# Samirez/Visual_odometry

Hardware: AMD Instinct MI355X
Metric: frame-pairs/sec (1280x720, 2000 ORB feats) (higher is better)
Workload: dtype u8+f32+f64; 1 GPU; seeded synthetic 1280x720 drone flight (256 distinct rendered views, closed loop), 2000 ORB features/frame, 8 levels = BASELINE config 2; chunk of 257 consecutive frames -> 256 pairs (k, k+1) per GPU per step, each frame detected once; detector=orb, distinct_rendered_frames=256, pair_stride=1, contexts_per_gpu=3, keypoint_order=cv2, poly_solver=fast, matcher=crosscheck, matcher_kernel=mfma_fp4, ransac=5-point, conf 0.99, 1 px, seed 2^64-1, <=1000 iters, parallelism=single GPU, pairs_ok_last_step=256

## Files before the change

include/vo_hip.h:

```cpp
#ifndef VO_HIP_H
#define VO_HIP_H
#include <stddef.h>
#include <stdint.h>

#ifdef __cplusplus
extern "C" {
#endif

#define VO_MAX_LEVELS 16

#define VO_OK                 0
#define VO_WARN_CAPACITY      1
#define VO_ERR_INVALID       -1
#define VO_ERR_HIP           -2
#define VO_ERR_TOO_FEW       -3
#define VO_ERR_NO_MODEL      -4
#define VO_ERR_NOT_CONFIGURED -5
#define VO_ERR_UNSUPPORTED    -7
#define VO_ERR_AMBIGUOUS      -6

typedef struct vo_ctx vo_ctx;

typedef struct {
    int32_t nfeatures;
// ... 26 lines not shown

int vo_set_pnp_refine(vo_ctx* ctx, int kind);

int vo_match_hamming(vo_ctx* ctx, const uint8_t* q, int nq, const uint8_t* t, int nt, int cross_check,
                     int32_t* qidx, int32_t* tidx, float* dist, int32_t* n_out);

int vo_match_l2(vo_ctx* ctx, const float* q, int nq, const float* t, int nt, int dim, int cross_check,
                int32_t* qidx, int32_t* tidx, float* dist, int32_t* n_out);

int vo_knn2_ratio_hamming(vo_ctx* ctx, const uint8_t* q, int nq, const uint8_t* t, int nt, double ratio,
                          int32_t* qidx, int32_t* tidx, float* dist, int32_t* n_out);
int vo_knn2_hamming(vo_ctx* ctx, const uint8_t* q, int nq, const uint8_t* t, int nt, int32_t* idx, float* dist);
int vo_knn2_l2(vo_ctx* ctx, const float* q, int nq, const float* t, int nt, int dim, int32_t* idx, float* dist);
int vo_knn2_ratio_l2(vo_ctx* ctx, const float* q, int nq, const float* t, int nt, int dim, double ratio,
                     int32_t* qidx, int32_t* tidx, float* dist, int32_t* n_out);

int vo_find_essential_ransac(vo_ctx* ctx, const double* p1, const double* p2, int M, const double* K,
                             double prob, double thresh_px, int max_iters, uint64_t seed,
                             double* E, uint8_t* mask, int32_t* n_inl, int32_t* n_models);

int vo_recover_pose(vo_ctx* ctx, const double* E, const double* p1, const double* p2, int M, const double* K,
                    double dist_thresh, double* R, double* t, uint8_t* mask, int32_t* n_good);

int vo_triangulate(vo_ctx* ctx, const double* P1, const double* P2, const double* x1, const double* x2,
                   int M, double* X);

int64_t vo_packed_pyramid_bytes(int h, int w, const vo_orb_params* params);
int vo_stage_pyramid(vo_ctx* ctx, const uint8_t* img, int h, int w, int channels, int row_stride,
                     const vo_orb_params* params, uint8_t* out_packed);
int vo_stage_fast_scores(vo_ctx* ctx, const uint8_t* img, int h, int w, int channels, int row_stride,
                         const vo_orb_params* params, uint8_t* out_packed);
int vo_stage_blur(vo_ctx* ctx, const uint8_t* img, int h, int w, int channels, int row_stride,
                  const vo_orb_params* params, uint8_t* out_packed);
int vo_stage_retain_best(vo_ctx* ctx, const float* response, int n, int n_points, int32_t* order, int32_t* n_out);
int vo_stage_five_point(vo_ctx* ctx, const double* x1, const double* x2, double* E , int32_t* n_models);

typedef struct {
    int32_t match_mode;
    double  ratio;
    double  ransac_prob;
    double  ransac_thresh;
    int32_t ransac_max_iters;
    uint64_t ransac_seed;
    double  pose_dist_thresh;
    int32_t want_points;
} vo_pair_opts;

typedef struct {
    int32_t n_kp1, n_kp2, n_match, n_inl, n_good, status, ransac_iters, reserved;
    double  R[9], t[3], E[9];
} vo_pair_result;

int vo_batch_configure(vo_ctx* ctx, int h, int w, const vo_orb_params* params, int max_frames, int max_pairs);
int vo_frames_upload(vo_ctx* ctx, const uint8_t* frames, int F, int row_stride, int64_t frame_stride, int first_slot);
int vo_frames_upload_async(vo_ctx* ctx, const uint8_t* frames, int F, int row_stride, int64_t frame_stride, int first_slot);
int vo_frames_upload_color(vo_ctx* ctx, const uint8_t* frames, int F, int channels, int row_stride,
                           int64_t frame_stride, int first_slot);
int vo_frames_detect(vo_ctx* ctx, int first_slot, int F);
int vo_frames_detect_async(vo_ctx* ctx, int first_slot, int F);
int vo_batch_kp_capacity(vo_ctx* ctx);
int  vo_host_alloc(size_t bytes, void** out);
void vo_host_free(void* p);
int vo_frame_features(vo_ctx* ctx, int slot, float* kp_xy, float* kp_size, float* kp_angle, float* kp_response,
                      int32_t* kp_octave, uint8_t* desc, int cap, int32_t* n_out);
int vo_pairs_run(vo_ctx* ctx, const int32_t* pair_slots, int B, const double* K, const vo_pair_opts* opts,
                 vo_pair_result* results, double* X, int32_t x_cap);
// ... 118 lines not shown
```

visual_odometry_amd/_lib.py:

```python
from __future__ import annotations

import ctypes as C
import os

import numpy as np

_HERE = os.path.dirname(os.path.abspath(__file__))
LIB_PATH = os.environ.get("VO_HIP_LIBRARY") or os.path.join(_HERE, "libvo_hip.so")

VO_OK, VO_WARN_CAPACITY = 0, 1
VO_ERR_INVALID, VO_ERR_HIP, VO_ERR_TOO_FEW, VO_ERR_NO_MODEL, VO_ERR_NOT_CONFIGURED, VO_ERR_AMBIGUOUS = -1, -2, -3, -4, -5, -6
VO_ERR_UNSUPPORTED = -7
VO_STAGE_COUNT = 28
VO_COMM_ID_BYTES, VO_RECORD_DOUBLES = 128, 16
VO_BA_MAX_CAMERAS, VO_BA_MAX_FREE = 64, 16


class OrbParams(C.Structure):
    _fields_ = [("nfeatures", C.c_int32), ("scale_factor", C.c_float), ("nlevels", C.c_int32),
                ("edge_threshold", C.c_int32), ("first_level", C.c_int32), ("wta_k", C.c_int32),
                ("score_type", C.c_int32), ("patch_size", C.c_int32), ("fast_threshold", C.c_int32)]


class SiftParams(C.Structure):
# ... 9 lines not shown

class BaOpts(C.Structure):
    _fields_ = [("iterations", C.c_int32), ("reserved", C.c_int32), ("huber_delta", C.c_double)]


class SlamOpts(C.Structure):
    _fields_ = [("pnp_iterations", C.c_int32), ("reproj_err", C.c_double), ("confidence", C.c_double), ("seed", C.c_uint64),
                ("max_point_norm", C.c_double), ("ba_iterations", C.c_int32), ("huber_delta", C.c_double),
                ("free_cameras", C.c_int32), ("filter_threshold", C.c_double), ("max_cameras", C.c_int32),
                ("snapshot_pair", C.c_int32), ("snapshot_stage", C.c_int32)]


PAIR_RESULT_DTYPE = np.dtype([("n_kp1", "<i4"), ("n_kp2", "<i4"), ("n_match", "<i4"), ("n_inl", "<i4"),
                              ("n_good", "<i4"), ("status", "<i4"), ("ransac_iters", "<i4"), ("reserved", "<i4"),
                              ("R", "<f8", (9,)), ("t", "<f8", (3,)), ("E", "<f8", (9,))], align=True)

_P = C.c_void_p
_SIGS = {
    "vo_create": (C.c_int, [C.c_int, C.POINTER(_P)]),
    "vo_destroy": (None, [_P]),
    "vo_last_error": (C.c_char_p, [_P]),
    "vo_version": (C.c_int, []),
    "vo_orb_detect_and_compute": (C.c_int, [_P, _P, C.c_int, C.c_int, C.c_int, C.c_int, _P, _P, _P, _P, _P, _P, _P, C.c_int, _P]),
    "vo_match_hamming": (C.c_int, [_P, _P, C.c_int, _P, C.c_int, C.c_int, _P, _P, _P, _P]),
    "vo_match_l2": (C.c_int, [_P, _P, C.c_int, _P, C.c_int, C.c_int, C.c_int, _P, _P, _P, _P]),
    "vo_knn2_ratio_hamming": (C.c_int, [_P, _P, C.c_int, _P, C.c_int, C.c_double, _P, _P, _P, _P]),
    "vo_find_essential_ransac": (C.c_int, [_P, _P, _P, C.c_int, _P, C.c_double, C.c_double, C.c_int, C.c_uint64, _P, _P, _P, _P]),
    "vo_recover_pose": (C.c_int, [_P, _P, _P, _P, C.c_int, _P, C.c_double, _P, _P, _P, _P]),
    "vo_triangulate": (C.c_int, [_P, _P, _P, _P, _P, C.c_int, _P]),
    "vo_packed_pyramid_bytes": (C.c_int64, [C.c_int, C.c_int, _P]),
    "vo_stage_pyramid": (C.c_int, [_P, _P, C.c_int, C.c_int, C.c_int, C.c_int, _P, _P]),
    "vo_stage_fast_scores": (C.c_int, [_P, _P, C.c_int, C.c_int, C.c_int, C.c_int, _P, _P]),
    "vo_stage_blur": (C.c_int, [_P, _P, C.c_int, C.c_int, C.c_int, C.c_int, _P, _P]),
    "vo_stage_five_point": (C.c_int, [_P, _P, _P, _P, _P]),
    "vo_batch_configure": (C.c_int, [_P, C.c_int, C.c_int, _P, C.c_int, C.c_int]),
    "vo_frames_upload": (C.c_int, [_P, _P, C.c_int, C.c_int, C.c_int64, C.c_int]),
    "vo_frames_upload_async": (C.c_int, [_P, _P, C.c_int, C.c_int, C.c_int64, C.c_int]),
    "vo_frames_upload_color": (C.c_int, [_P, _P, C.c_int, C.c_int, C.c_int, C.c_int64, C.c_int]),
    "vo_frames_detect": (C.c_int, [_P, C.c_int, C.c_int]),
    "vo_frames_detect_async": (C.c_int, [_P, C.c_int, C.c_int]),
    "vo_batch_kp_capacity": (C.c_int, [_P]),
    "vo_host_alloc": (C.c_int, [C.c_size_t, C.POINTER(_P)]),
    "vo_host_free": (None, [_P]),
    "vo_frame_features": (C.c_int, [_P, C.c_int, _P, _P, _P, _P, _P, _P, C.c_int, _P]),
    "vo_pairs_run": (C.c_int, [_P, _P, C.c_int, _P, _P, _P, _P, C.c_int32]),
    "vo_pairs_run_async": (C.c_int, [_P, _P, C.c_int, _P, _P, _P, _P, C.c_int32]),
    "vo_sync": (C.c_int, [_P]),
    "vo_set_matcher_kernel": (C.c_int, [_P, C.c_int]),
    "vo_set_poly_solver": (C.c_int, [_P, C.c_int]),
    "vo_set_pnp_refine": (C.c_int, [_P, C.c_int]),
    "vo_set_keypoint_order": (C.c_int, [_P, C.c_int]),
    "vo_stage_retain_best": (C.c_int, [_P, _P, C.c_int, C.c_int, _P, _P]),
    "vo_detect_after": (C.c_int, [_P, _P]),
    "vo_knn2_hamming": (C.c_int, [_P, _P, C.c_int, _P, C.c_int, _P, _P]),
    "vo_knn2_l2": (C.c_int, [_P, _P, C.c_int, _P, C.c_int, C.c_int, _P, _P]),
    "vo_knn2_ratio_l2": (C.c_int, [_P, _P, C.c_int, _P, C.c_int, C.c_int, C.c_double, _P, _P, _P, _P]),
    "vo_tracks_pnp_batch": (C.c_int, [_P, C.c_int, _P, C.c_int, C.c_double, C.c_double, C.c_uint64, C.c_double, _P, _P, _P, _P, _P]),
    "vo_slam_chain": (C.c_int, [_P, C.c_int, _P, _P, _P, _P, _P, _P, _P, _P, _P, _P, _P, _P, _P]),
    "vo_slam_map_size": (C.c_int, [_P, C.c_int, _P, _P, _P]),
    "vo_slam_map": (C.c_int, [_P, C.c_int, _P, _P, _P, _P, _P, _P, _P, _P]),
    "vo_slam_chains": (C.c_int, [_P, C.c_int, _P, _P, _P, C.c_int, _P, _P, _P, _P, _P, _P, _P, _P, _P, _P, _P]),
    "vo_slam_chains_map_size": (C.c_int, [_P, C.c_int, C.c_int, _P, _P, _P]),
    "vo_slam_chains_map": (C.c_int, [_P, C.c_int, C.c_int, _P, _P, _P, _P, _P, _P, _P, _P]),
    "vo_comm_unique_id": (C.c_int, [_P]),
    "vo_comm_init": (C.c_int, [_P, _P, C.c_int, C.c_int]),
    "vo_comm_destroy": (C.c_int, [_P]),
# ... 205 lines not shown
```

visual_odometry_amd/csrc/orb_kernels.hip:

```cpp
#include "vo_internal.h"
#include <type_traits>
#include <float.h>
#include <stdlib.h>

__constant__ int8_t c_pattern[256 * 4] = {
#include "orb_pattern.inc"
};
__constant__ int c_umax[16] = {15, 15, 15, 15, 14, 14, 14, 13, 13, 12, 11, 10, 9, 8, 6, 3};
__constant__ int c_gauss7[7] = {18, 34, 49, 55, 49, 34, 18};


typedef short vo_s16x2 __attribute__((ext_vector_type(2)));
typedef unsigned short vo_u16x2 __attribute__((ext_vector_type(2)));
__device__ __forceinline__ uint32_t pk_sub16(uint32_t a, uint32_t b)
{
    return __builtin_bit_cast(uint32_t, __builtin_bit_cast(vo_s16x2, a) - __builtin_bit_cast(vo_s16x2, b));
}
__device__ __forceinline__ uint32_t pk_add16(uint32_t a, uint32_t b)
{
    return __builtin_bit_cast(uint32_t, __builtin_bit_cast(vo_s16x2, a) + __builtin_bit_cast(vo_s16x2, b));
}
__device__ __forceinline__ uint32_t pk_min16(uint32_t a, uint32_t b)
{
    return __builtin_bit_cast(uint32_t, __builtin_elementwise_min(__builtin_bit_cast(vo_s16x2, a), __builtin_bit_cast(vo_s16x2, b)));
// ... 114 lines not shown
        const int dx = dx0 + b;
        uint32_t v = 0;
        if (dx < dst.w) {
            uint32_t h0, h1;
            if (dx < tab.min_x)       { h0 = (uint32_t)s0[0] << 8; h1 = (uint32_t)s1[0] << 8; }
            else if (dx >= tab.max_x) { h0 = (uint32_t)s0[src.w - 1] << 8; h1 = (uint32_t)s1[src.w - 1] << 8; }
            else {
                const int xo = tab.xofs[dx];
                const uint32_t c1 = tab.xc1[dx], c0 = 256 - c1;
                h0 = c0 * s0[xo] + c1 * s0[xo + 1];
                h1 = c0 * s1[xo] + c1 * s1[xo + 1];
            }
            v = edge ? (h0 + 128u) >> 8 : (h0 * w0 + h1 * w1 + 32768u) >> 16;
            v = v > 255u ? 255u : v;
        }
        out |= v << (8 * b);
    }
    *(uint32_t*)(dp + (size_t)dy * dst.stride + dx0) = out;
}

template <int I, int N, typename F>
__device__ __forceinline__ void unroll_while(int n, F& f)
{
    if constexpr (I < N) {
        if (I < n) { f(std::integral_constant<int, I>{}); unroll_while<I + 1, N>(n, f); }
    }
}

#ifndef RS3_AHEAD
#define RS3_AHEAD 4
#endif
__global__ __launch_bounds__(RS2_THREADS) void k_resize_direct(uint8_t* pyr, int frame_bytes, LevelGeom src, LevelGeom dst, ResizeTab tab)
{
    const int f = blockIdx.z, tid = threadIdx.x, lane = tid & 63, wave = __builtin_amdgcn_readfirstlane(tid >> 6);
    const int tiles_x = (dst.w + RS2_WW - 1) / RS2_WW;
    const int bid = xcd_tile(blockIdx.x, gridDim.x);
    const int tx = bid % tiles_x, ty = bid / tiles_x;
    const int x0 = tx * RS2_WW, y0 = ty * RS2_TH;
    const int dy0 = y0 + wave * RS2_WH, dy1 = min(dy0 + RS2_WH, dst.h);
    if (dy0 >= dst.h) return;
    const uint8_t* sp = pyr + (size_t)f * frame_bytes + src.off;
    const int dx = x0 + 4 * lane;
    int o[4], c1[4];
#pragma unroll
    for (int i = 0; i < 4; i++) { const int xi = min(dx + i, dst.w - 1); o[i] = tab.xofs[xi]; c1[i] = tab.xc1[xi]; }
    static_assert(RS2_WH <= 64, "one lane per destination row of the strip");
    const int li = min(dy0 + lane, dst.h - 1);
    const int yo_l = tab.yofs[li];
    const uint32_t yw1 = tab.yc1[li];
    const int yc_l = (int)((256u - yw1) | (yw1 << 16));
    const int yo_first = __builtin_amdgcn_readlane(yo_l, 0), yo_last = __builtin_amdgcn_readlane(yo_l, dy1 - 1 - dy0);
    const int base = o[0] & ~3, sh = o[0] - base;
    const uint32_t q1 = (uint32_t)(o[1] - o[0]), q2 = (uint32_t)(o[2] - o[0]), q3 = (uint32_t)(o[3] - o[0]);
    const uint32_t sel_ae = 0x0c000c00u | (q2 << 16), sel_ao = 0x0c000c00u | q1 | (q3 << 16);
    const uint32_t sel_be = sel_ae + 0x00010001u, sel_bo = sel_ao + 0x00010001u;
    const uint32_t c1e = (uint32_t)c1[0] | ((uint32_t)c1[2] << 16), c1o = (uint32_t)c1[1] | ((uint32_t)c1[3] << 16);
    const int r_first = yo_first, r_end = yo_last + 2;
    static_assert((RS2_WH * 127 + 99) / 100 + 3 <= 32, "the emit mask of a strip fits 32 bits");
    uint32_t emask = dy0 + lane < dy1 ? 1u << (yo_l + 1 - r_first) : 0u;
#pragma unroll
    for (int d = 1; d < RS2_WH; d <<= 1) emask |= (uint32_t)__shfl_xor((int)emask, d, 64);
    emask = (uint32_t)__builtin_amdgcn_readfirstlane((int)emask);
    const __amdgpu_buffer_rsrc_t drs = __builtin_amdgcn_make_buffer_rsrc(pyr + (size_t)f * frame_bytes + dst.off, 0, dst.stride * dst.h, 0x00020000);
    uint32_t out = (uint32_t)(dy0 * dst.stride + dx);
    const bool col_ok = dx < dst.stride;
    const int hmax = src.h - 1;
    uint32_t w[RS3_AHEAD][3];
#pragma unroll
    for (int u = 0; u < RS3_AHEAD; u++) {
        const uint32_t* q = (const uint32_t*)(sp + ((uint32_t)(min(r_first + u, hmax) * src.stride) + (uint32_t)base));
        w[u][0] = q[0]; w[u][1] = q[1]; w[u][2] = q[2];
    }
    int dyi = 0;
    uint32_t pe = 0, po = 0;
    const int nrows = r_end - r_first;
    constexpr int RS3_MAXR = (RS2_WH * 127 + 99) / 100 + 3;
    auto row = [&](auto ic) {
        constexpr int i = decltype(ic)::value, u = i % RS3_AHEAD;
        const uint32_t w0 = w[u][0], w1 = w[u][1], w2 = w[u][2];
        {
            const uint32_t* q = (const uint32_t*)(sp + ((uint32_t)(min(r_first + i + RS3_AHEAD, hmax) * src.stride) + (uint32_t)base));
            w[u][0] = q[0]; w[u][1] = q[1]; w[u][2] = q[2];
        }
        const uint32_t x0w = __builtin_amdgcn_alignbyte(w1, w0, (uint32_t)sh), x1w = __builtin_amdgcn_alignbyte(w2, w1, (uint32_t)sh);
        const uint32_t a_e = __builtin_amdgcn_perm(x1w, x0w, sel_ae), a_o = __builtin_amdgcn_perm(x1w, x0w, sel_ao);
        const uint32_t b_e = __builtin_amdgcn_perm(x1w, x0w, sel_be), b_o = __builtin_amdgcn_perm(x1w, x0w, sel_bo);
        const vo_u16x2 h_e = __builtin_bit_cast(vo_u16x2, c1e) * __builtin_bit_cast(vo_u16x2, pk_sub16(b_e, a_e)) + __builtin_bit_cast(vo_u16x2, a_e << 8);
        const vo_u16x2 h_o = __builtin_bit_cast(vo_u16x2, c1o) * __builtin_bit_cast(vo_u16x2, pk_sub16(b_o, a_o)) + __builtin_bit_cast(vo_u16x2, a_o << 8);
        const uint32_t ce = __builtin_bit_cast(uint32_t, h_e), co = __builtin_bit_cast(uint32_t, h_o);
        {
            const bool emit = emask & 1u;
            emask >>= 1;
            const vo_u16x2 wv = __builtin_bit_cast(vo_u16x2, __builtin_amdgcn_readlane(yc_l, dyi));
            const uint32_t d0 = __builtin_amdgcn_udot2(__builtin_bit_cast(vo_u16x2, __builtin_amdgcn_perm(ce, pe, 0x05040100u)), wv, 32768u, false);
            const uint32_t d2 = __builtin_amdgcn_udot2(__builtin_bit_cast(vo_u16x2, __builtin_amdgcn_perm(ce, pe, 0x07060302u)), wv, 32768u, false);
            const uint32_t d1 = __builtin_amdgcn_udot2(__builtin_bit_cast(vo_u16x2, __builtin_amdgcn_perm(co, po, 0x05040100u)), wv, 32768u, false);
            const uint32_t d3 = __builtin_amdgcn_udot2(__builtin_bit_cast(vo_u16x2, __builtin_amdgcn_perm(co, po, 0x07060302u)), wv, 32768u, false);
            const uint32_t t01 = __builtin_amdgcn_perm(d1, d0, 0x0c0c0602u), t23 = __builtin_amdgcn_perm(d3, d2, 0x0c0c0602u);
            __builtin_amdgcn_raw_buffer_store_b32(__builtin_amdgcn_perm(t23, t01, 0x05040100u), drs, col_ok && emit ? out : 0xfffffff0u, 0, 0);
            out += emit ? (uint32_t)dst.stride : 0u;
            dyi += emit ? 1 : 0;
        }
        pe = ce; po = co;
    };
    unroll_while<0, RS3_MAXR>(nrows, row);
}

void launch_resize(hipStream_t s, uint8_t* pyr, const PyrGeom& g, int level, const ResizeTab& tab, int F)
{
    const LevelGeom& d = g.lv[level];
    if (tab.direct) {
        dim3 grid(((d.w + RS2_WW - 1) / RS2_WW) * ((d.h + RS2_TH - 1) / RS2_TH), 1, F);
        hipLaunchKernelGGL(k_resize_direct, grid, dim3(RS2_THREADS), 0, s, pyr, g.frame_bytes, g.lv[level - 1], d, tab);
        return;
// ... 1084 lines not shown
        if (EDGE) { bd_fix(a0, a1, a2, e); bd_fix(b0, b1, b2, e); }
        bd_hpass(a0, a1, a2, h0); bd_hpass(b0, b1, b2, h1);
#pragma unroll
        for (int c = 0; c < 4; c++) q[c] = h0[c] | (h1[c] << 16);
    };
#pragma unroll
    for (int u = 0; u < BD_AHEAD; u++) fetch(u, W[u]);
#pragma unroll
    for (int k = 0; k < 3; k++) {
        hstep(W[k % BD_AHEAD], Q[k % 4]);
        fetch(k + BD_AHEAD, W[k % BD_AHEAD]);
    }
    uint32_t orow = (uint32_t)(y0 * lv.stride);
    for (int m0 = 0; m0 < nsteps; m0 += 4) {
#pragma unroll
        for (int j = 0; j < 4; j++) {
            const int m = m0 + j;
            if (m >= nsteps) break;
            constexpr int K0 = 3;
            const int ki = (K0 + j) % 4, wi = (K0 + j) % BD_AHEAD;
            hstep(W[wi], Q[ki]);
            fetch(K0 + m + BD_AHEAD, W[wi]);
            const uint32_t r0 = bd_vrow<false>(Q[(ki + 1) % 4], Q[(ki + 2) % 4], Q[(ki + 3) % 4], Q[ki]);
            const uint32_t r1 = bd_vrow<true>(Q[(ki + 1) % 4], Q[(ki + 2) % 4], Q[(ki + 3) % 4], Q[ki]);
            __builtin_amdgcn_raw_buffer_store_b32(r0, drs, col_ok ? (uint32_t)x + orow : 0xfffffff0u, 0, 0);
            __builtin_amdgcn_raw_buffer_store_b32(r1, drs, col_ok && 2 * m + 1 < nout ? (uint32_t)x + orow + (uint32_t)lv.stride : 0xfffffff0u, 0, 0);
            orow += 2u * (uint32_t)lv.stride;
        }
    }
}

__global__ __launch_bounds__(256) void k_blur_direct(const uint8_t* pyr, uint8_t* blur, PyrGeom g, int total)
{
    const int f = blockIdx.y, lane = threadIdx.x & 63, wave = __builtin_amdgcn_readfirstlane(threadIdx.x >> 6);
    const int wt = xcd_tile(blockIdx.x, gridDim.x) * 4 + wave;
    if (wt >= total) return;
    int l = 0, first = 0;
    for (;;) {
        const int nt = ((g.lv[l].stride + 255) / 256) * ((g.lv[l].h + BD_R - 1) / BD_R);
        if (wt < first + nt || l + 1 == g.nlevels) break;
        first += nt; l++;
    }
    const LevelGeom lv = g.lv[l];
    const int ntx = (lv.stride + 255) / 256, tile = wt - first;
    const int x0 = (tile % ntx) * 256, y0 = (tile / ntx) * BD_R;
    const int x = x0 + 4 * lane;
    const uint8_t* img = pyr + (size_t)f * g.frame_bytes + lv.off;
    const int xb = min(max(x - 4, 0), lv.stride - 12);
    BdEdge e;
    e.left = x0 == 0; e.right = x0 + 256 + 8 > lv.w;
    e.shl = x == 0; e.shr = x - 4 > lv.stride - 12 && x < lv.stride;
    {
        const int d = lv.w - x;
        e.s1 = d == 1 ? 0x01020304u : d == 2 ? 0x03040504u : d == 3 ? 0x05060504u : 0x07060504u;
        e.s2 = d == 2 ? 0x0c0c0c02u : d == 3 ? 0x0c0c0304u : 0x0c040506u;
        e.s3 = d == 5 ? 0x01020304u : d == 6 ? 0x03040504u : 0x07060504u;
        e.use_t = d >= 2 && d <= 4;
    }
    const __amdgpu_buffer_rsrc_t drs = __builtin_amdgcn_make_buffer_rsrc(blur + (size_t)f * g.frame_bytes + lv.off, 0, lv.stride * lv.h, 0x00020000);
    const bool col_ok = x < lv.stride;
    const int nout = min(BD_R, lv.h - y0);
    const int nsteps = (nout + 1) / 2;
    const bool inside = y0 >= 3 && y0 - 3 + 2 * (nsteps + 3 + BD_AHEAD) <= lv.h, edge = e.left || e.right;
    if (inside && !edge) bd_strip<true, false>(img, lv, drs, x, xb, y0, nout, nsteps, col_ok, e);
    else if (inside) bd_strip<true, true>(img, lv, drs, x, xb, y0, nout, nsteps, col_ok, e);
    else if (!edge) bd_strip<false, false>(img, lv, drs, x, xb, y0, nout, nsteps, col_ok, e);
    else bd_strip<false, true>(img, lv, drs, x, xb, y0, nout, nsteps, col_ok, e);
}

void launch_blur(hipStream_t s, const uint8_t* pyr, uint8_t* blur, const PyrGeom& g, int F)
{
    bool direct = true;
    int total = 0;
    for (int l = 0; l < g.nlevels; l++) {
        direct = direct && g.lv[l].w >= 16 && g.lv[l].h >= 8;
        total += ((g.lv[l].stride + 255) / 256) * ((g.lv[l].h + BD_R - 1) / BD_R);
    }
    if (direct) { hipLaunchKernelGGL(k_blur_direct, dim3((total + 3) / 4, F), dim3(256), 0, s, pyr, blur, g, total); return; }
    hipLaunchKernelGGL(k_blur, dim3(g.btiles_total, F), dim3(256), 0, s, pyr, blur, g);
}

__device__ __forceinline__ uint32_t brief_expand4(uint32_t nib)
{
    const uint32_t m = (nib * 0x00204081u) & 0x01010101u;
    return 0x81818181u ^ (m * 0xfeu);
}

__device__ __forceinline__ uint32_t brief_expand8_fp4(uint32_t b)
{
    uint32_t w = (b | (b << 12)) & 0x000F000Fu;
    w = (w | (w << 6)) & 0x03030303u;
    w = (w | (w << 3)) & 0x11111111u;
    return 0xAAAAAAAAu ^ (w << 3);
}

__global__ __launch_bounds__(256) void k_brief_trig(PyrGeom g, FrameFeat ff)
{
    const int f = blockIdx.y, k = blockIdx.x * 256 + threadIdx.x;
    if (k >= min(ff.kp_count[f], g.kp_cap)) return;
    const size_t ki = (size_t)f * g.kp_cap + k;
// ... 103 lines not shown
```

visual_odometry_amd/csrc/vo_api.hip:

```cpp
#include "vo_internal.h"
#include <float.h>
#include <math.h>
#include <stdio.h>
#include <stdlib.h>
#include <string.h>
#include <vector>
#include <type_traits>
#include <algorithm>

#define MAX_EVENTS 384

struct DevList {
    struct Entry { void* p; bool pinned; };
    std::vector<Entry> ptrs;
    DevList() = default;
    DevList(const DevList&) = delete;
    DevList& operator=(DevList&& o) noexcept { if (this != &o) { release(); ptrs.swap(o.ptrs); } return *this; }
    ~DevList() { release(); }
    template <typename T> hipError_t alloc(T** p, size_t n) { return keep(hipMalloc((void**)p, (n ? n : 1) * sizeof(T)), (void**)p, false); }
    template <typename T> hipError_t alloc_pinned(T** p, size_t n)
    {
        return keep(hipHostMalloc((void**)p, (n ? n : 1) * sizeof(T), hipHostMallocDefault), (void**)p, true);
    }
    void release()
// ... 216 lines not shown
    const double sf = (double)p->scale_factor;
    const float factor = (float)(1.0 / sf);
    float nd = p->nfeatures * (1 - factor) / (1 - (float)pow((double)factor, (double)L));
    int sum = 0, off = 0, ft = 0, bt = 0, co = 0, sc = 0, dt = 0;
    for (int l = 0; l < L; l++) {
        LevelGeom& lv = g->lv[l];
        lv.scale = (float)pow(sf, (double)l);
        lv.w = cv_round_f((float)w / lv.scale);
        lv.h = cv_round_f((float)h / lv.scale);
        if (lv.w < 1 || lv.h < 1) FAIL(VO_ERR_INVALID, "pyramid level %d is empty (%dx%d input)", l, w, h);
        if (lv.w > 65535 || lv.h > 65535) FAIL(VO_ERR_INVALID, "image too large");
        lv.stride = align_up(lv.w, 64);
        lv.off = off;
        off += lv.stride * lv.h;
        if (l < L - 1) { lv.quota = cv_round_f(nd); sum += lv.quota; nd *= factor; }
        else lv.quota = p->nfeatures - sum > 0 ? p->nfeatures - sum : 0;
        lv.fox = (p->edge_threshold - 1) & ~15; lv.foy = p->edge_threshold;
        const int iw = lv.w - p->edge_threshold - lv.fox, ih = lv.h - p->edge_threshold - lv.foy;
        const int trows = iw > 0 && ih > 0 ? (ih + FAST_TH - 1) / FAST_TH : 0;
        lv.ftile_base = ft; lv.ftiles_x = trows > 0 ? (iw + FAST_TW - 1) / FAST_TW : 0;
        ft += lv.ftiles_x * trows;
        lv.dtile_base = dt; lv.dtiles_x = (lv.w + FAST_TW - 1) / FAST_TW;
        dt += lv.dtiles_x * ((lv.h + FAST_TH - 1) / FAST_TH);
        lv.btile_base = bt; lv.btiles_x = (lv.w + BLUR_TW - 1) / BLUR_TW;
        bt += lv.btiles_x * ((lv.h + BLUR_TH - 1) / BLUR_TH);
        const int want = p->score_type == 0 ? 2 * lv.quota : lv.quota;
        lv.sel_chunk_base = sc;
        sc += trows;
        lv.cand_off = co;
        lv.cand_cap = align_up(want + (want > 1024 ? want : 1024), 8);
        co += lv.cand_cap;
    }
    g->frame_bytes = align_up(off, 256);
    g->ftiles_total = ft; g->btiles_total = bt; g->dtiles_total = dt;
    g->cand_total = co;
    g->sel_chunks_total = sc;
    g->kp_cap = align_up(p->nfeatures + (p->nfeatures / 8 > 256 ? p->nfeatures / 8 : 256), 8);
    return VO_OK;
}

static void build_lin_tab(int ssize, int dsize, int* ofs, uint16_t* c1, int* pmin, int* pmax)
{
    const double inv_scale = (double)dsize / (double)ssize;
    const double scale = 1.0 / inv_scale;
    int minofst = 0, maxofst = dsize;
    for (int val = 0; val < dsize; val++) {
        volatile double fval = scale * ((double)val + 0.5);
        fval = fval - 0.5;
        const double fv = fval;
        const int ival = cv_floor_d(fv);
        ofs[val] = 0; c1[val] = 0;
        if (ival >= 0 && ssize > 1) {
            if (ival < ssize - 1) {
                ofs[val] = ival;
                volatile double fr = fv - (double)ival;
                fr = fr * 256.0;
                c1[val] = (uint16_t)lrint((double)fr);
            } else {
                ofs[val] = ssize - 1;
                if (val < maxofst) maxofst = val;
            }
        } else if (val + 1 > minofst) minofst = val + 1;
    }
    *pmin = minofst; *pmax = maxofst;
}

// ... 466 lines not shown
struct KpArrays { const float *xy, *size, *angle, *resp; const int* octave; const uint8_t* desc; int desc_bytes; };

static int download_keypoints(vo_ctx* ctx, const KpArrays& d, size_t first, int n, float* kp_xy, float* kp_size, float* kp_angle,
                              float* kp_response, int32_t* kp_octave, uint8_t* desc)
{
    if (n <= 0) return VO_OK;
    if (kp_xy) HIPCHK(hipMemcpy(kp_xy, d.xy + first * 2, (size_t)n * 2 * sizeof(float), hipMemcpyDeviceToHost));
    if (kp_size) HIPCHK(hipMemcpy(kp_size, d.size + first, (size_t)n * sizeof(float), hipMemcpyDeviceToHost));
    if (kp_angle) HIPCHK(hipMemcpy(kp_angle, d.angle + first, (size_t)n * sizeof(float), hipMemcpyDeviceToHost));
    if (kp_response) HIPCHK(hipMemcpy(kp_response, d.resp + first, (size_t)n * sizeof(float), hipMemcpyDeviceToHost));
    if (kp_octave) HIPCHK(hipMemcpy(kp_octave, d.octave + first, (size_t)n * sizeof(int), hipMemcpyDeviceToHost));
    if (desc) HIPCHK(hipMemcpy(desc, d.desc + first * d.desc_bytes, (size_t)n * d.desc_bytes, hipMemcpyDeviceToHost));
    return VO_OK;
}

extern "C" int vo_frame_features(vo_ctx* ctx, int slot, float* kp_xy, float* kp_size, float* kp_angle, float* kp_response,
                                 int32_t* kp_octave, uint8_t* desc, int cap, int32_t* n_out)
{
    if (!ctx) return VO_ERR_INVALID;
    if (!ctx->configured) FAIL(VO_ERR_NOT_CONFIGURED, "vo_batch_configure has not been called");
    if (slot < 0 || slot >= ctx->max_frames || !n_out) FAIL(VO_ERR_INVALID, "bad slot");
    HIPCHK(hipSetDevice(ctx->device));
    const FrameFeat& ff = ctx->ff;
    int n = 0, flags = 0;
    HIPCHK(hipStreamSynchronize(ctx->stream));
    HIPCHK(hipMemcpy(&n, ff.kp_count + slot, sizeof(int), hipMemcpyDeviceToHost));
    HIPCHK(hipMemcpy(&flags, ff.flags + slot, sizeof(int), hipMemcpyDeviceToHost));
    int warn = (flags & 1) ? VO_WARN_CAPACITY : VO_OK;
    if (n > cap) { n = cap; warn = VO_WARN_CAPACITY; }
    *n_out = n;
    const int rc = download_keypoints(ctx, {ff.kp_xy, ff.kp_size, ff.kp_angle, ff.kp_resp, ff.kp_level, ff.desc, 32}, (size_t)slot * ctx->g.kp_cap, n,
                                      kp_xy, kp_size, kp_angle, kp_response, kp_octave, desc);
    return rc ? rc : warn;
}

static int load_single(vo_ctx* ctx, const uint8_t* img, int h, int w, int channels, int row_stride, const vo_orb_params* params)
{
    if (!img || h < 1 || w < 1) FAIL(VO_ERR_INVALID, "bad image");
    if (channels != 1 && channels != 3 && channels != 4) FAIL(VO_ERR_INVALID, "channels must be 1, 3 or 4");
    if (row_stride < w * channels) FAIL(VO_ERR_INVALID, "row_stride too small");
    int mf = ctx->configured ? ctx->max_frames : 1, mp = ctx->configured ? ctx->max_pairs : 1;
    int rc = vo_batch_configure(ctx, h, w, params, mf, mp);
    if (rc) return rc;
    if (channels == 1) return vo_frames_upload(ctx, img, 1, row_stride, 0, 0);
    const size_t bytes = (size_t)row_stride * h;
    rc = ctx->staging.grow(ctx, bytes); if (rc) return rc;
    HIPCHK(hipMemcpyAsync(ctx->staging.p, img, bytes, hipMemcpyHostToDevice, ctx->stream));
    { StageTimer t(ctx, ST_GRAY); launch_gray(ctx->stream, ctx->staging.p, channels, row_stride, 0, ctx->pyr, ctx->g, 1); }
    HIPCHK(hipStreamSynchronize(ctx->stream));
    return VO_OK;
}

extern "C" int vo_orb_detect_and_compute(vo_ctx* ctx, const uint8_t* img, int h, int w, int channels, int row_stride,
                                         const vo_orb_params* params, float* kp_xy, float* kp_size, float* kp_angle,
                                         float* kp_response, int32_t* kp_octave, uint8_t* desc, int cap, int32_t* n_out)
{
    if (!ctx) return VO_ERR_INVALID;
    if (!n_out || cap < 0) FAIL(VO_ERR_INVALID, "bad output arguments");
    int rc = check_params(ctx, params);
    if (rc) return rc;
    rc = load_single(ctx, img, h, w, channels, row_stride, params);
    if (rc) return rc;
    rc = vo_frames_detect(ctx, 0, 1);
    if (rc) return rc;
    return vo_frame_features(ctx, 0, kp_xy, kp_size, kp_angle, kp_response, kp_octave, desc, cap, n_out);
}
// ... 2183 lines not shown
```

visual_odometry_amd/csrc/vo_internal.h:

```cpp
#pragma once
#include <hip/hip_runtime.h>
#include <stdint.h>
#include "../../include/vo_hip.h"

enum {
    ST_GRAY = 0, ST_RESIZE, ST_FAST, ST_SELECT_FAST, ST_HARRIS, ST_SELECT_HARRIS, ST_ANGLE,
    ST_BLUR, ST_BRIEF, ST_MATCH_NN, ST_MATCH_SELECT, ST_RANSAC, ST_POSE, ST_TRIANGULATE,
    ST_MISC, ST_RESERVED, ST_SIFT_SCALE, ST_SIFT_EXTREMA, ST_SIFT_ORIENT, ST_SIFT_SORT, ST_SIFT_DESC, ST_CV2_ORDER, ST_GATHER, ST_RESERVED2,
    ST_SLAM_PREPARE, ST_SLAM_BA, ST_SLAM_FILTER, ST_SLAM_LIMIT
};

struct LevelGeom {
    int w, h, stride, off;
    int quota;
    float scale;
    int ftile_base, ftiles_x;
    int fox, foy;
    int dtile_base, dtiles_x;
    int btile_base, btiles_x;
    int cand_off, cand_cap;
    int sel_chunk_base;
};

struct PyrGeom {
    int nlevels, frame_bytes;
    int edge, fast_thr, score_type, nfeatures;
    int ftiles_total, btiles_total, dtiles_total;
    int cand_total, kp_cap;
    int sel_chunks_total;
    LevelGeom lv[VO_MAX_LEVELS];
};

#define RS2_WW 256
#define RS2_WH 16
#ifndef RS2_WAVES
#define RS2_WAVES 4
#endif
#define RS2_THREADS (64 * RS2_WAVES)
#define RS2_TH (RS2_WAVES * RS2_WH)

struct ResizeTab {
    const int* xofs; const uint16_t* xc1;
    const int* yofs; const uint16_t* yc1;
    int min_x, max_x, min_y, max_y;
    int direct;
};

#ifndef FAST_TW
#define FAST_TW 112
#endif
#ifndef FAST_TH
#define FAST_TH 20
#endif
#define BLUR_TW 128
#ifndef BLUR_TH
// ... 256 lines not shown
```

visual_odometry_amd/frontend.py:

```python
from __future__ import annotations

import ctypes as C

import numpy as np

from . import _lib
from .detector import make_params
from .geometry import OPENCV_RNG_SEED

MATCH_CROSSCHECK, MATCH_RATIO, MATCH_CROSSCHECK_LEGACY, MATCH_NEAREST = 0, 1, 2, 3


class FrontEnd:
    def __init__(self, height, width, max_frames, max_pairs, nfeatures=500, nlevels=8, device=0, ctx=None,
                 keypoint_order="cv2", detector="orb", kp_cap=0, **det_kw):
        self.ctx = ctx or _lib.Context(device)
        self.h, self.w = int(height), int(width)
        self.max_frames, self.max_pairs = int(max_frames), int(max_pairs)
        self.detector = detector
        c = self.ctx
        if detector == "sift":
            self.params = _lib.SiftParams(0, int(det_kw.pop("nOctaveLayers", 3)), float(det_kw.pop("contrastThreshold", 0.04)),
                                          float(det_kw.pop("edgeThreshold", 10.0)), float(det_kw.pop("sigma", 1.6)))
            if det_kw:
# ... 44 lines not shown
            out = np.empty((f.shape[0], self.h, self.w) if f.ndim == 3 else (f.shape[0], self.h, self.w, cn), np.uint8)
        c = self.ctx
        c.check(c.lib.vo_frames_ingest(c.handle, f.ctypes.data, f.shape[0], f.shape[1], f.shape[2], cn, f.strides[1],
                                       f.strides[0], int(first_slot), _lib.ptr(out)))
        return out

    def ingest_jpeg(self, buffers, first_slot=0, want_resized=False):
        from .ingest import _packed
        blob, offs, _keep = _packed(buffers)
        n = len(offs) - 1
        out = np.empty((n, self.h, self.w, 3), np.uint8) if want_resized else None
        c = self.ctx
        rc = c.lib.vo_frames_ingest_jpeg(c.handle, blob.ctypes.data, offs.ctypes.data, n, int(first_slot), _lib.ptr(out))
        if rc == _lib.VO_ERR_UNSUPPORTED:
            raise NotImplementedError(c.last_error())
        c.check(rc)
        return out

    def detect(self, first_slot, count, wait=True, after=None):
        c = self.ctx
        if after is not None and after is not self:
            c.check(c.lib.vo_detect_after(c.handle, after.ctx.handle))
        fn = c.lib.vo_frames_detect if wait else c.lib.vo_frames_detect_async
        self._warn_capacity(c.check(fn(c.handle, int(first_slot), int(count))))

    def features(self, slot):
        sift = self.detector == "sift"
        kp = _lib.KeypointBuffers(self.kp_cap, 128 if sift else 32)
        c = self.ctx
        fn = c.lib.vo_frame_features_sift if sift else c.lib.vo_frame_features
        rc = c.check(fn(c.handle, int(slot), *kp.args()))
        return kp.result(rc, np.float32 if sift else None)

    def set_sift_rows(self, slot, rows, xy=None):
        if self.detector != "sift":
            raise ValueError("set_sift_rows needs detector='sift'")
        r = np.asarray(rows)
        if r.dtype != np.uint8 or r.ndim != 2 or r.shape[1] != 128:
            raise ValueError("rows must be [n, 128] uint8")
        r = np.ascontiguousarray(r)
        p = None
        if xy is not None:
            p = np.ascontiguousarray(xy, dtype=np.float32)
            if p.shape != (len(r), 2):
                raise ValueError("xy must be [n, 2]")
        c = self.ctx
        c.check(c.lib.vo_stage_sift_rows(c.handle, int(slot), r.ctypes.data, len(r), _lib.ptr(p)))

    def make_opts(self, match_mode=MATCH_CROSSCHECK, ratio=0.75, prob=0.99, thresh=1.0, max_iters=1000,
                  seed=OPENCV_RNG_SEED, dist_thresh=50.0, want_points=False):
        return _lib.PairOpts(int(match_mode), float(ratio), float(prob), float(thresh), int(max_iters), int(seed),
                             float(dist_thresh), int(bool(want_points)))

    def run_pairs(self, pair_slots, K, opts=None, want_points=False, wait=True):
        ps = np.ascontiguousarray(pair_slots, dtype=np.int32).reshape(-1, 2)
        B = len(ps)
        K = np.ascontiguousarray(K, dtype=np.float64).reshape(3, 3)
        opts = opts or self.make_opts(want_points=want_points)
        if B > self.max_pairs:
            raise ValueError(f"{B} pairs > max_pairs={self.max_pairs}")
        res = self._res.array[:B]
        X = None
        if opts.want_points:
            if self._X is None:
                self._X = _lib.PinnedArray((self.max_pairs, 4, self.kp_cap), np.float64)
            X = self._X.array[:B]
# ... 152 lines not shown
```

Before: 95830 frame-pairs/s.

## Pack multiple frames into last partial column tile in resize and blur kernels

In the pyramid resize and blur kernels, the rightmost column tile of each level usually covers only a few lanes' worth of pixels. When it does, several frames are now packed into one wavefront, with lane groups assigned to different frames, so fewer idle lanes are launched. Frame offsets are folded into the load and buffer-store addresses, and the buffer range is widened to span the packed frames. A debug API to download a pyramid or blur level for verification is also added. This adds index arithmetic and per-lane frame bounds checks. It assumes the grid launch sizes still cover all frames, since the launch code is unchanged.

```diff
diff --git a/include/vo_hip.h b/include/vo_hip.h
--- a/include/vo_hip.h
+++ b/include/vo_hip.h
@@ -82,6 +82,7 @@
                          const vo_orb_params* params, uint8_t* out_packed);
 int vo_stage_blur(vo_ctx* ctx, const uint8_t* img, int h, int w, int channels, int row_stride,
                   const vo_orb_params* params, uint8_t* out_packed);
+int vo_stage_batch_level(vo_ctx* ctx, int slot, int which , int level, uint8_t* out);
 int vo_stage_retain_best(vo_ctx* ctx, const float* response, int n, int n_points, int32_t* order, int32_t* n_out);
 int vo_stage_five_point(vo_ctx* ctx, const double* x1, const double* x2, double* E , int32_t* n_models);
 
diff --git a/visual_odometry_amd/_lib.py b/visual_odometry_amd/_lib.py
--- a/visual_odometry_amd/_lib.py
+++ b/visual_odometry_amd/_lib.py
@@ -65,6 +65,7 @@
     "vo_stage_pyramid": (C.c_int, [_P, _P, C.c_int, C.c_int, C.c_int, C.c_int, _P, _P]),
     "vo_stage_fast_scores": (C.c_int, [_P, _P, C.c_int, C.c_int, C.c_int, C.c_int, _P, _P]),
     "vo_stage_blur": (C.c_int, [_P, _P, C.c_int, C.c_int, C.c_int, C.c_int, _P, _P]),
+    "vo_stage_batch_level": (C.c_int, [_P, C.c_int, C.c_int, C.c_int, _P]),
     "vo_stage_five_point": (C.c_int, [_P, _P, _P, _P, _P]),
     "vo_batch_configure": (C.c_int, [_P, C.c_int, C.c_int, _P, C.c_int, C.c_int]),
     "vo_frames_upload": (C.c_int, [_P, _P, C.c_int, C.c_int, C.c_int64, C.c_int]),
diff --git a/visual_odometry_amd/csrc/orb_kernels.hip b/visual_odometry_amd/csrc/orb_kernels.hip
--- a/visual_odometry_amd/csrc/orb_kernels.hip
+++ b/visual_odometry_amd/csrc/orb_kernels.hip
@@ -170,25 +170,33 @@
 #endif
 __global__ __launch_bounds__(RS2_THREADS) void k_resize_direct(uint8_t* pyr, int frame_bytes, LevelGeom src, LevelGeom dst, ResizeTab tab)
 {
-    const int f = blockIdx.z, tid = threadIdx.x, lane = tid & 63, wave = __builtin_amdgcn_readfirstlane(tid >> 6);
+    const int F = gridDim.z, tid = threadIdx.x, lane = tid & 63, wave = __builtin_amdgcn_readfirstlane(tid >> 6);
     const int tiles_x = (dst.w + RS2_WW - 1) / RS2_WW;
     const int bid = xcd_tile(blockIdx.x, gridDim.x);
     const int tx = bid % tiles_x, ty = bid / tiles_x;
     const int x0 = tx * RS2_WW, y0 = ty * RS2_TH;
+    const int pk = tx == tiles_x - 1 ? dst.fpack_log2 : 0;
+    const int f0 = (int)blockIdx.z << pk;
+    if (f0 >= F) return;
     const int dy0 = y0 + wave * RS2_WH, dy1 = min(dy0 + RS2_WH, dst.h);
     if (dy0 >= dst.h) return;
-    const uint8_t* sp = pyr + (size_t)f * frame_bytes + src.off;
-    const int dx = x0 + 4 * lane;
+    const int nfr = min(1 << pk, F - f0);
+    const int grp = lane >> (6 - pk), li = lane - (grp << (6 - pk));
+    const bool f_ok = grp < nfr;
+    const uint32_t fo_ld = (uint32_t)(min(grp, nfr - 1) * frame_bytes), fo_st = (uint32_t)(grp * frame_bytes);
+    const uint8_t* sp = pyr + (size_t)f0 * frame_bytes + src.off;
+    const int dx = x0 + 4 * li;
     int o[4], c1[4];
 #pragma unroll
     for (int i = 0; i < 4; i++) { const int xi = min(dx + i, dst.w - 1); o[i] = tab.xofs[xi]; c1[i] = tab.xc1[xi]; }
     static_assert(RS2_WH <= 64, "one lane per destination row of the strip");
-    const int li = min(dy0 + lane, dst.h - 1);
-    const int yo_l = tab.yofs[li];
-    const uint32_t yw1 = tab.yc1[li];
+    const int ri = min(dy0 + lane, dst.h - 1);
+    const int yo_l = tab.yofs[ri];
+    const uint32_t yw1 = tab.yc1[ri];
     const int yc_l = (int)((256u - yw1) | (yw1 << 16));
     const int yo_first = __builtin_amdgcn_readlane(yo_l, 0), yo_last = __builtin_amdgcn_readlane(yo_l, dy1 - 1 - dy0);
-    const int base = o[0] & ~3, sh = o[0] - base;
+    const int sh = o[0] & 3;
+    const uint32_t base = (uint32_t)(o[0] & ~3) + fo_ld;
     const uint32_t q1 = (uint32_t)(o[1] - o[0]), q2 = (uint32_t)(o[2] - o[0]), q3 = (uint32_t)(o[3] - o[0]);
     const uint32_t sel_ae = 0x0c000c00u | (q2 << 16), sel_ao = 0x0c000c00u | q1 | (q3 << 16);
     const uint32_t sel_be = sel_ae + 0x00010001u, sel_bo = sel_ao + 0x00010001u;
@@ -199,14 +207,15 @@
 #pragma unroll
     for (int d = 1; d < RS2_WH; d <<= 1) emask |= (uint32_t)__shfl_xor((int)emask, d, 64);
     emask = (uint32_t)__builtin_amdgcn_readfirstlane((int)emask);
-    const __amdgpu_buffer_rsrc_t drs = __builtin_amdgcn_make_buffer_rsrc(pyr + (size_t)f * frame_bytes + dst.off, 0, dst.stride * dst.h, 0x00020000);
-    uint32_t out = (uint32_t)(dy0 * dst.stride + dx);
-    const bool col_ok = dx < dst.stride;
+    const __amdgpu_buffer_rsrc_t drs = __builtin_amdgcn_make_buffer_rsrc(pyr + (size_t)f0 * frame_bytes + dst.off, 0,
+                                                                         (nfr - 1) * frame_bytes + dst.stride * dst.h, 0x00020000);
+    uint32_t out = (uint32_t)(dy0 * dst.stride + dx) + fo_st;
+    const bool col_ok = dx < dst.stride && f_ok;
     const int hmax = src.h - 1;
     uint32_t w[RS3_AHEAD][3];
 #pragma unroll
     for (int u = 0; u < RS3_AHEAD; u++) {
-        const uint32_t* q = (const uint32_t*)(sp + ((uint32_t)(min(r_first + u, hmax) * src.stride) + (uint32_t)base));
+        const uint32_t* q = (const uint32_t*)(sp + ((uint32_t)(min(r_first + u, hmax) * src.stride) + base));
         w[u][0] = q[0]; w[u][1] = q[1]; w[u][2] = q[2];
     }
     int dyi = 0;
@@ -217,7 +226,7 @@
         constexpr int i = decltype(ic)::value, u = i % RS3_AHEAD;
         const uint32_t w0 = w[u][0], w1 = w[u][1], w2 = w[u][2];
         {
-            const uint32_t* q = (const uint32_t*)(sp + ((uint32_t)(min(r_first + i + RS3_AHEAD, hmax) * src.stride) + (uint32_t)base));
+            const uint32_t* q = (const uint32_t*)(sp + ((uint32_t)(min(r_first + i + RS3_AHEAD, hmax) * src.stride) + base));
             w[u][0] = q[0]; w[u][1] = q[1]; w[u][2] = q[2];
         }
         const uint32_t x0w = __builtin_amdgcn_alignbyte(w1, w0, (uint32_t)sh), x1w = __builtin_amdgcn_alignbyte(w2, w1, (uint32_t)sh);
@@ -1368,7 +1377,7 @@
 
 __global__ __launch_bounds__(256) void k_blur_direct(const uint8_t* pyr, uint8_t* blur, PyrGeom g, int total)
 {
-    const int f = blockIdx.y, lane = threadIdx.x & 63, wave = __builtin_amdgcn_readfirstlane(threadIdx.x >> 6);
+    const int F = gridDim.y, lane = threadIdx.x & 63, wave = __builtin_amdgcn_readfirstlane(threadIdx.x >> 6);
     const int wt = xcd_tile(blockIdx.x, gridDim.x) * 4 + wave;
     if (wt >= total) return;
     int l = 0, first = 0;
@@ -1378,11 +1387,18 @@
         first += nt; l++;
     }
     const LevelGeom lv = g.lv[l];
-    const int ntx = (lv.stride + 255) / 256, tile = wt - first;
-    const int x0 = (tile % ntx) * 256, y0 = (tile / ntx) * BD_R;
-    const int x = x0 + 4 * lane;
-    const uint8_t* img = pyr + (size_t)f * g.frame_bytes + lv.off;
-    const int xb = min(max(x - 4, 0), lv.stride - 12);
+    const int ntx = (lv.stride + 255) / 256, tile = wt - first, tcol = tile % ntx;
+    const int x0 = tcol * 256, y0 = (tile / ntx) * BD_R;
+    const int pk = tcol == ntx - 1 ? lv.fpack_log2 : 0;
+    const int f0 = (int)blockIdx.y << pk;
+    if (f0 >= F) return;
+    const int nfr = min(1 << pk, F - f0);
+    const int grp = lane >> (6 - pk), li = lane - (grp << (6 - pk));
+    const bool f_ok = grp < nfr;
+    const uint32_t fo_ld = (uint32_t)(min(grp, nfr - 1) * g.frame_bytes), fo_st = (uint32_t)(grp * g.frame_bytes);
+    const int x = x0 + 4 * li;
+    const uint8_t* img = pyr + (size_t)f0 * g.frame_bytes + lv.off;
+    const int xb = (int)((uint32_t)min(max(x - 4, 0), lv.stride - 12) + fo_ld);
     BdEdge e;
     e.left = x0 == 0; e.right = x0 + 256 + 8 > lv.w;
     e.shl = x == 0; e.shr = x - 4 > lv.stride - 12 && x < lv.stride;
@@ -1393,15 +1409,17 @@
         e.s3 = d == 5 ? 0x01020304u : d == 6 ? 0x03040504u : 0x07060504u;
         e.use_t = d >= 2 && d <= 4;
     }
-    const __amdgpu_buffer_rsrc_t drs = __builtin_amdgcn_make_buffer_rsrc(blur + (size_t)f * g.frame_bytes + lv.off, 0, lv.stride * lv.h, 0x00020000);
-    const bool col_ok = x < lv.stride;
+    const __amdgpu_buffer_rsrc_t drs = __builtin_amdgcn_make_buffer_rsrc(blur + (size_t)f0 * g.frame_bytes + lv.off, 0,
+                                                                         (nfr - 1) * g.frame_bytes + lv.stride * lv.h, 0x00020000);
+    const bool col_ok = x < lv.stride && f_ok;
+    const int xs = (int)((uint32_t)x + fo_st);
     const int nout = min(BD_R, lv.h - y0);
     const int nsteps = (nout + 1) / 2;
     const bool inside = y0 >= 3 && y0 - 3 + 2 * (nsteps + 3 + BD_AHEAD) <= lv.h, edge = e.left || e.right;
-    if (inside && !edge) bd_strip<true, false>(img, lv, drs, x, xb, y0, nout, nsteps, col_ok, e);
-    else if (inside) bd_strip<true, true>(img, lv, drs, x, xb, y0, nout, nsteps, col_ok, e);
-    else if (!edge) bd_strip<false, false>(img, lv, drs, x, xb, y0, nout, nsteps, col_ok, e);
-    else bd_strip<false, true>(img, lv, drs, x, xb, y0, nout, nsteps, col_ok, e);
+    if (inside && !edge) bd_strip<true, false>(img, lv, drs, xs, xb, y0, nout, nsteps, col_ok, e);
+    else if (inside) bd_strip<true, true>(img, lv, drs, xs, xb, y0, nout, nsteps, col_ok, e);
+    else if (!edge) bd_strip<false, false>(img, lv, drs, xs, xb, y0, nout, nsteps, col_ok, e);
+    else bd_strip<false, true>(img, lv, drs, xs, xb, y0, nout, nsteps, col_ok, e);
 }
 
 void launch_blur(hipStream_t s, const uint8_t* pyr, uint8_t* blur, const PyrGeom& g, int F)
diff --git a/visual_odometry_amd/csrc/vo_api.hip b/visual_odometry_amd/csrc/vo_api.hip
--- a/visual_odometry_amd/csrc/vo_api.hip
+++ b/visual_odometry_amd/csrc/vo_api.hip
@@ -272,6 +272,7 @@
         co += lv.cand_cap;
     }
     g->frame_bytes = align_up(off, 256);
+    for (int l = 0; l < L; l++) g->lv[l].fpack_log2 = frame_pack_log2(g->lv[l].stride, g->frame_bytes);
     g->ftiles_total = ft; g->btiles_total = bt; g->dtiles_total = dt;
     g->cand_total = co;
     g->sel_chunks_total = sc;
@@ -804,6 +805,20 @@
     const int rc = download_keypoints(ctx, {ff.kp_xy, ff.kp_size, ff.kp_angle, ff.kp_resp, ff.kp_level, ff.desc, 32}, (size_t)slot * ctx->g.kp_cap, n,
                                       kp_xy, kp_size, kp_angle, kp_response, kp_octave, desc);
     return rc ? rc : warn;
+}
+
+extern "C" int vo_stage_batch_level(vo_ctx* ctx, int slot, int which, int level, uint8_t* out)
+{
+    if (!ctx) return VO_ERR_INVALID;
+    if (!ctx->configured || ctx->detector != 0) FAIL(VO_ERR_NOT_CONFIGURED, "vo_batch_configure has not been called");
+    if (slot < 0 || slot >= ctx->max_frames) FAIL(VO_ERR_INVALID, "bad slot");
+    if (which < 0 || which > 1 || level < 0 || level >= ctx->g.nlevels || !out) FAIL(VO_ERR_INVALID, "bad level or image");
+    HIPCHK(hipSetDevice(ctx->device));
+    HIPCHK(hipStreamSynchronize(ctx->stream));
+    const LevelGeom& lv = ctx->g.lv[level];
+    const uint8_t* src = (which ? ctx->blur : ctx->pyr) + (size_t)slot * ctx->g.frame_bytes + lv.off;
+    HIPCHK(hipMemcpy2D(out, lv.w, src, lv.stride, lv.w, lv.h, hipMemcpyDeviceToHost));
+    return VO_OK;
 }
 
 static int load_single(vo_ctx* ctx, const uint8_t* img, int h, int w, int channels, int row_stride, const vo_orb_params* params)
diff --git a/visual_odometry_amd/csrc/vo_internal.h b/visual_odometry_amd/csrc/vo_internal.h
--- a/visual_odometry_amd/csrc/vo_internal.h
+++ b/visual_odometry_amd/csrc/vo_internal.h
@@ -20,7 +20,15 @@
     int btile_base, btiles_x;
     int cand_off, cand_cap;
     int sel_chunk_base;
-};
+    int fpack_log2;
+};
+
+static inline int frame_pack_log2(int stride, int frame_bytes)
+{
+    const int n = (stride % 256) / 4;
+    const int lg = n == 0 || n > 32 ? 0 : n > 16 ? 1 : 2;
+    return ((int64_t)frame_bytes << lg) <= 0x7fffffff ? lg : 0;
+}
 
 struct PyrGeom {
     int nlevels, frame_bytes;
diff --git a/visual_odometry_amd/frontend.py b/visual_odometry_amd/frontend.py
--- a/visual_odometry_amd/frontend.py
+++ b/visual_odometry_amd/frontend.py
@@ -100,6 +100,18 @@
         rc = c.check(fn(c.handle, int(slot), *kp.args()))
         return kp.result(rc, np.float32 if sift else None)
 
+    def level_image(self, slot, level, blurred=False):
+        if self.detector != "orb":
+            raise ValueError("level_image needs detector='orb'")
+        if not 0 <= int(level) < self.params.nlevels:
+            raise ValueError(f"level must be in 0..{self.params.nlevels - 1}")
+        scale = np.float32(float(self.params.scale_factor) ** int(level))
+        lw, lh = (int(np.rint(np.float32(v) / scale)) for v in (self.w, self.h))
+        out = np.empty(self.h * self.w, np.uint8)
+        c = self.ctx
+        c.check(c.lib.vo_stage_batch_level(c.handle, int(slot), int(bool(blurred)), int(level), out.ctypes.data))
+        return out[:lh * lw].reshape(lh, lw).copy()
+
     def set_sift_rows(self, slot, rows, xy=None):
         if self.detector != "sift":
             raise ValueError("set_sift_rows needs detector='sift'")
```

Result: no change. 96130 frame-pairs/s, median of 4 (+0.3%).
